# tsinghua-fib-lab/PIML

Measured on AMD Instinct MI355X. Metric: agent-pair force evals/sec + simulated steps/sec, 4096-agent GC scene, higher is better.
Workload: dtype f32

## Files before the change

### include/piml_hip_tuning.h

```cpp
#ifndef PIML_HIP_TUNING_H
#define PIML_HIP_TUNING_H

#include "piml_hip.h"

#ifdef __cplusplus
extern "C" {
#endif

int piml_timer_create(void** event);
int piml_timer_record(void* event, void* stream);
int piml_timer_elapsed_ms(void* start, void* stop, float* ms);
int piml_timer_destroy(void* event);

int piml_trace_begin(void);
int piml_trace_mark(const char* name, void* stream);
int piml_trace_end(char* names, int names_cap, float* us, int us_cap);

int piml_probe_arith(const float* rx, const float* ry, const float* hx, const float* hy,
                     float* dist, float* cosv, int n, void* stream);

long long piml_encoder_split_tiles(long long tiles);
long long piml_encoder_split_tiles_train(long long tiles);
int piml_encoder_products(int split_bf16);
int piml_rowdecoder_products(int split_bf16);
int piml_encoder_dw2(int layer_split);
int piml_encoder_fused_bwd(int on);
int piml_encoder_sums_bwd(int form);
int piml_encoder_sums_dec_slots(int on);
int piml_encoder_compact_rows(int on);
int piml_pinnsf_streams_init(void);

#ifdef __cplusplus
}
#endif
#endif
```

### piml_amd/_lib.py

```python
import ctypes
import os

import torch

_HERE = os.path.dirname(os.path.abspath(__file__))
LIB_PATH = os.environ.get('PIML_LIB') or os.path.join(_HERE, 'libpiml_hip.so')
ABI_VERSION = 35
COMPACT_MAX_AGENTS = 16384
COMPACT_SLOTS = 256

_lib = None

_i, _f, _p, _z = ctypes.c_int, ctypes.c_float, ctypes.c_void_p, ctypes.c_size_t
_ll = ctypes.c_longlong
_d = ctypes.c_double


class EncoderBranch(ctypes.Structure):
    _fields_ = [('x', _p), ('rows', _ll), ('in_dim', _i), ('k', _i),
                ('w1', _p), ('b1', _p), ('w2', _p), ('b2', _p), ('w3', _p), ('b3', _p),
                ('scale', _f), ('h1', _p), ('h2', _p), ('msgs', _p), ('g_pooled', _p), ('g_msgs', _p),
                ('g2', _p), ('g1', _p), ('g_x', _p), ('partials', _p), ('grads', _p), ('packed', _p), ('relu_mask', _p),
                ('keep_bits', _p), ('drop_state', _p), ('drop_p', _f), ('sum_a', _p), ('sum_b', _p),
                ('nbr_idx', _p), ('plan', _p)]
# ... 176 lines not shown
    'piml_train_step_tail_bwd': [_p, _ll, _p, _p, _p, _p, _ll, _p, _p, _i, _i, _i, _i, _f, _p, _p, _p, _p, _p, _f, _i, _i, _p, _p, _p, _p],
    'piml_pinnsf_epilogue_fwd': [_p, _p, _p, _z, _f, _p, _p],
    'piml_pinnsf_epilogue_bwd': [_p, _p, _z, _f, _p, _p],
    'piml_pinnsf_epilogue_ksum_fwd': [_p, _i, _p, _i, _p, _z, _f, _p, _p],
    'piml_pinnsf_epilogue_ksum_bwd': [_p, _p, _z, _f, _i, _i, _p, _p, _p, _p],
    'piml_pinnsf_epilogue_agentnorm_fwd': [_p, _p, _p, _i, _i, _f, _p, _p],
    'piml_pinnsf_epilogue_ksum_agentnorm_fwd': [_p, _i, _p, _i, _p, _i, _i, _f, _p, _p],
    'piml_pinnsf_epilogue_agentnorm_bwd': [_p, _p, _i, _i, _f, _p, _p],
    'piml_self_features_fwd': [_p, _i, _p, _p, _z, _p, _p],
    'piml_self_features_bwd': [_p, _z, _p, _p, _p, _p],
    'piml_colsum_blocks': [_z, _i],
    'piml_act_bwd_colsum': [_p, _p, _z, _i, _p, _p, _p, _p],
    'piml_sum_leading': [_p, _i, _z, _p, _p],
    'piml_act_bwd_colsum_stage1': [_p, _p, _z, _i, _p, _p, _p, _p],
    'piml_layer_reduce': [_p, _i, _z, _p, _p, _i, _i, _p, _p],
    'piml_scale_ksum_fwd': [_p, _p, _z, _i, _i, _f, _p, _p, _p, _p],
    'piml_ksum_blocks': [_z, _i],
    'piml_scale_ksum_bwd': [_p, _p, _z, _i, _i, _f, _p, _p, _p, _p],
    'piml_dropout_keep_bits': [_p, _ll, _i, _f, _i, _p, _p],
    'piml_timer_create': [ctypes.POINTER(_p)],
    'piml_timer_record': [_p, _p],
    'piml_timer_elapsed_ms': [_p, _p, ctypes.POINTER(_f)],
    'piml_timer_destroy': [_p],
    'piml_trace_begin': [],
    'piml_trace_mark': [ctypes.c_char_p, _p],
    'piml_trace_end': [ctypes.c_char_p, _i, ctypes.POINTER(_f), _i],
    'piml_probe_arith': [_p, _p, _p, _p, _p, _p, _i, _p],
    'piml_encoder_partial_floats': [],
    'piml_encoder_pack_floats': [],
    'piml_encoder_split_tiles': [_ll],
    'piml_encoder_split_tiles_train': [_ll],
    'piml_multi_copy': [ctypes.POINTER(_p), ctypes.POINTER(_p), ctypes.POINTER(_z), _i, _p],
    'piml_rollout_prologue': [_p] * 8 + [_i] * 4 + [_p] * 11 + [_p],
    'piml_rollout_losses_blocks': [_i, _i],
    'piml_rollout_losses': [_p, _p, _ll, _p, _p, _p, _p, _p, _i, _i, _i, _f, _p, _p, _p, _p, _p, _p, _p],
    'piml_rollout_losses_bwd': [_p, _p, _p, _p, _p, _p, _ll, _p, _p],
    'piml_rollout_losses_frames': [_p, _p, _ll, _p, _p, ctypes.POINTER(_p), _i, _p, _i, _i, _i, _f, _f, _f, _p, _p, _p, _p, _p, _p, _p],
    'piml_rollout_losses_frames_bwd': [_p, _p, _p, _p, _f, _f, _p, _p, _p, _ll, _p, _p],
    'piml_collision_pred_loss_blocks': [_ll, _i],
    'piml_collision_pred_loss': [ctypes.POINTER(_p), ctypes.POINTER(_p), _i, _ll, _i, _i, _p, _i, _i, _f, _p, _p, _p, _p, _p],
    'piml_collision_pred_loss_bwd': [_p, _p, _ll, _p, _p],
    'piml_adam_tickets': [],
    'piml_adam_step': [ctypes.POINTER(_p)] * 5 + [ctypes.POINTER(_ll), _i, ctypes.c_double, ctypes.c_double, ctypes.c_double, ctypes.c_double, ctypes.c_double, _p, _p],
    'piml_pointwise_losses_blocks': [_ll, _ll, _i],
    'piml_pointwise_losses': [_p, _p, _ll, _ll, _p, _ll, _f, _p, _i, _p, _p, _p, _p, _p],
    'piml_p2p_alloc': [_z, ctypes.POINTER(_p)],
    'piml_p2p_free': [_p],
    'piml_p2p_export': [_p, _p],
    'piml_p2p_open': [_p, ctypes.POINTER(_p)],
    'piml_p2p_close': [_p],
    'piml_p2p_copy': [_p, _p, _z, _p],
    'piml_allgather_state_p2p': [_p, _z, _i, _i, ctypes.POINTER(_p), ctypes.POINTER(_p), ctypes.c_uint, ctypes.c_uint, _p, _p],
    'piml_encoder_products': [_i],
    'piml_rowdecoder_products': [_i],
    'piml_encoder_dw2': [_i],
    'piml_encoder_fused_bwd': [_i],
    'piml_encoder_sums_bwd': [_i],
    'piml_encoder_sums_dec_slots': [_i],
    'piml_encoder_compact_rows': [_i],
    'piml_encoder_pack': [ctypes.POINTER(EncoderBranch), _i, _p],
    'piml_encoder_workgroups': [ctypes.POINTER(EncoderBranch), _i, ctypes.POINTER(_i)],
    'piml_encoder_fwd': [ctypes.POINTER(EncoderBranch), _i, _p],
    'piml_encoder_fwd_packed': [ctypes.POINTER(EncoderBranch), _i, _p],
    'piml_encoder_bwd': [ctypes.POINTER(EncoderBranch), _i, _p],
    'piml_encoder_bwd_acc': [ctypes.POINTER(EncoderBranch), _i, _i, _p],
    'piml_encoder_ksum': [_p, _ll, _i, _p, _p],
    'piml_decoder_pack_floats': [],
    'piml_decoder_partial_floats': [],
    'piml_decoder_workgroups': [_ll],
    'piml_decoder_fwd': [ctypes.POINTER(DecoderBranch), _i, _p, _f, _p, _p],
    'piml_decoder_bwd': [ctypes.POINTER(DecoderBranch), _i, _p, _p, _f, _p, _p],
    'piml_rowdecoder_slots': [_ll],
    'piml_rowdecoder_fwd': [ctypes.POINTER(DecoderBranch), _i, _p],
    'piml_rowdecoder_fwd_packed': [ctypes.POINTER(DecoderBranch), _i, _p],
    'piml_rowdecoder_bwd': [ctypes.POINTER(DecoderBranch), _i, _p],
    'piml_rowdecoder_bwd_acc': [ctypes.POINTER(DecoderBranch), _i, _i, _p],
    'piml_collision_head_pack_floats': [],
    'piml_collision_head_fwd': [_p, _ll, _p, _p, _p, _p, _p, _p, _p],
    'piml_head64_partial_floats': [],
    'piml_head64_slots': [_ll],
    'piml_head64_fwd': [ctypes.POINTER(Head64), _p],
    'piml_head64_bwd': [ctypes.POINTER(Head64), _p],
    'piml_head64_bwd_acc': [ctypes.POINTER(Head64), _i, _p],
    'piml_corrector_partial_floats': [_i],
    'piml_corrector_slots': [_i, _ll, _i],
    'piml_corrector_fwd': [ctypes.POINTER(Corrector), _p],
    'piml_corrector_bwd': [ctypes.POINTER(Corrector), _i, _p],
    'piml_pinnsf_pool_h2_ok': [ctypes.POINTER(EncoderBranch), _i],
    'piml_pinnsf_pool_train_ok': [ctypes.POINTER(EncoderBranch), _i],
    'piml_pinnsf_pool_msgs_ok': [ctypes.POINTER(EncoderBranch), _i],
    'piml_pinnsf_streams_init': [],
    'piml_pinnsf_pack_flush': [],
    'piml_pinnsf_slot_sums_flush': [],
    'piml_pinnsf_pack': [ctypes.POINTER(EncoderBranch), ctypes.POINTER(DecoderBranch), _i, ctypes.POINTER(CollisionHead),
                         _i, _p],
    'piml_pinnsf_fwd': [ctypes.POINTER(EncoderBranch), ctypes.POINTER(DecoderBranch), _i, ctypes.POINTER(CollisionHead),
                        _p, _f, _p, _i, _p],
    'piml_pinnsf_bwd': [ctypes.POINTER(EncoderBranch), ctypes.POINTER(DecoderBranch), _i, _p, _p, _f, _p, _i, _p],
    'piml_comm_available': [],
    'piml_comm_unique_id': [_p],
    'piml_comm_init': [ctypes.POINTER(_p), _i, _i, _p],
    'piml_comm_destroy': [_p],
    'piml_allgather_state': [_p, _p, _z, _p, _p],
    'piml_reducescatter_grad': [_p, _p, _p, _z, _p],
    'piml_allreduce_sum': [_p, _p, _z, _p],
    'piml_relfeat_fwd_self': [_p, _p, _p, _p, _i, _p, _p, _p, _i, _i, _i, _i, _i, _i, _i, _f, _f, _f, _f, _p, _p, _p, _p, _p, _p, _p],
# ... 173 lines not shown
```

### piml_amd/csrc/network.hip

```cpp
#include <cstdio>
#include <cstdlib>
#include <mutex>

#include "common.hpp"
#include "pack.hpp"
#include "reduce.hpp"
#include "stages.hpp"
#include "trace.hpp"

namespace piml {

namespace {

struct Side {
    hipStream_t s[2] = {nullptr, nullptr};
    hipEvent_t ev[6] = {};
    bool ok = false;
};

constexpr int kMaxDevices = 64;
Side g_side[kMaxDevices];
std::mutex g_mu;

int side_streams(Side** out) {
    int dev = 0;
    if (hipError_t e = hipGetDevice(&dev)) return e;
    if (dev < 0 || dev >= kMaxDevices) return hipErrorInvalidDevice;
    std::lock_guard<std::mutex> lock(g_mu);
    Side& S = g_side[dev];
    if (!S.ok) {
        for (auto& s : S.s)
            if (hipError_t e = hipStreamCreateWithFlags(&s, hipStreamNonBlocking)) return e;
        for (auto& ev : S.ev)
            if (hipError_t e = hipEventCreateWithFlags(&ev, hipEventDisableTiming)) return e;
        S.ok = true;
    }
    *out = &S;
    return hipSuccess;
}

int edge(hipStream_t from, hipStream_t to, hipEvent_t ev) {
    if (hipError_t e = hipEventRecord(ev, from)) return e;
    return hipStreamWaitEvent(to, ev, 0);
}

#define PIML_TRY(x)                                                                        \
    do {                                                                                   \
        if (int e_ = (x)) {                                                                \
            fprintf(stderr, "libpiml_hip: %s -> %d (%s:%d)\n", #x, e_, __FILE__, __LINE__); \
            return e_;                                                                     \
        }                                                                                  \
    } while (0)

}

__global__ __launch_bounds__(256) void pinnsf_pack_kernel(PackAll A) {
    __shared__ double red[256];
    pack_block(A, (int)blockIdx.x, 256, red);
}

int launch_pack(const PackAll& A, hipStream_t s) {
    hipLaunchKernelGGL(pinnsf_pack_kernel, dim3((unsigned)pack_blocks_total(A, 256)), dim3(256), 0, s, A);
    trace_mark("pinnsf_pack", s);
    return hipGetLastError();
}

__global__ __launch_bounds__(256) void pinnsf_reduce_kernel(ReduceAll A) { reduce_launch_block(A, (int)blockIdx.x); }

int launch_slot_sums(const ReduceAll& R, hipStream_t s) {
    hipLaunchKernelGGL(pinnsf_reduce_kernel, dim3((unsigned)reduce_launch_blocks(R)), dim3(256), 0, s, R);
    return hipGetLastError();
}

__global__ __launch_bounds__(256) void pinnsf_unfold_kernel(ReduceAll R) { unfold_block(R, (int)(blockIdx.y * kUnfoldBlocks + blockIdx.x)); }

static int launch_unfold_now(const ReduceAll& R, hipStream_t s) {
    if (R.nunf <= 0) return hipSuccess;
    hipLaunchKernelGGL(pinnsf_unfold_kernel, dim3(kUnfoldBlocks, (unsigned)R.nunf), dim3(256), 0, s, R);
    trace_mark("pinnsf_unfold", s);
    return hipGetLastError();
}

namespace {
struct PendingUnfold {
    ReduceAll R;
    hipStream_t stream = nullptr;
    bool valid = false, deferring = false;
};
PendingUnfold g_pending_unfold[kMaxDevices];
PendingUnfold* pending_unfold_entry() {
    int dev = 0;
    if (hipGetDevice(&dev) || dev < 0 || dev >= kMaxDevices) return nullptr;
    return &g_pending_unfold[dev];
}
bool same_unfold(const ReduceAll& a, const ReduceAll& b) {
    if (a.nunf != b.nunf) return false;
    for (int i = 0; i < a.nunf; ++i)
        if (a.unf[i].dgrads != b.unf[i].dgrads || a.unf[i].dw1_out != b.unf[i].dw1_out || a.unf[i].egrads != b.unf[i].egrads ||
            a.unf[i].w1 != b.unf[i].w1 || a.unf[i].w3 != b.unf[i].w3 || a.unf[i].b3 != b.unf[i].b3 || a.unf[i].k != b.unf[i].k ||
            a.unf[i].scale != b.unf[i].scale)
            return false;
    return true;
}
}

ReduceAll unfold_begin(const ReduceAll& R, hipStream_t s, UnfoldTail* t) {
    ReduceAll out = R;
    out.unf_blocks = 0;
    t->go = false;
    if (R.nunf <= 0) return out;
    PendingUnfold* P = pending_unfold_entry();
// ... 376 lines not shown
```

### piml_amd/csrc/reduce.hpp

```cpp
#pragma once
#include <hip/hip_runtime.h>

#include "pack.hpp"

namespace piml {

struct ReduceSet {
    const float* parts;
    float* grads;
    int slots, lanes, split, off0, off1;
    const int* dev_slots;
};
struct UnfoldSet {
    const float* dgrads;
    const float *w1, *w3, *b3;
    float scale;
    int k;
    float* dw1_out;
    float* egrads;
};
constexpr int REDUCE_SETS = 8;
struct ReduceAll {
    ReduceSet set[REDUCE_SETS];
    int nsets;
// ... 69 lines not shown
    const int y = bid / A.gx, x = bid - y * A.gx;
    const ReduceSet S = A.set[y];
    if (x * 16 < S.lanes) sum_slots_16x16_at(x, S.parts, S.grads, S.dev_slots ? *S.dev_slots : S.slots, S.lanes, S.split, S.off0, S.off1, A.accumulate != 0);
}
__device__ __forceinline__ void reduce_launch_block(const ReduceAll& A, int bid) {
    if (bid < A.unf_blocks) unfold_block(A, bid);
    else reduce_block(A, bid - A.unf_blocks);
}
__host__ __device__ inline int reduce_launch_blocks(const ReduceAll& A) { return A.unf_blocks + A.gx * A.nsets; }

struct PackAll {
    piml_encoder_branch enc[2];
    piml_decoder_branch dec[2];
    piml_collision_head head;
    int nbr, has_head;
    int has_fold;
    int skip_f32;
};
constexpr int ENC_LIVE_X3 = PACK_FLOATS - 2 * 32768;
__host__ __device__ inline int enc_set_elems(const PackAll& A) { return A.skip_f32 ? ENC_LIVE_X3 : PACK_FLOATS; }
__host__ __device__ inline int pack_elems_total(const PackAll& A) {
    return A.nbr * (enc_set_elems(A) + DEC_PACK_PLAIN) + (A.has_head ? HEAD_PACK_PLAIN : 0);
}

__device__ __forceinline__ void pack_flat(const PackAll& A, int t) {
    const int ne = enc_set_elems(A);
    for (int y = 0; y < A.nbr; ++y) {
        if (t < ne) {
            int e = t;
            if (A.skip_f32) e = t < PACK_FWD - 32768 ? t + 32768 : t + 2 * 32768;
            const piml_encoder_branch& J = A.enc[y];
            J.packed[e] = pack_value(J, e);
            return;
        }
        t -= ne;
    }
    for (int y = 0; y < A.nbr; ++y) {
        if (t < DEC_PACK_PLAIN) {
            const piml_decoder_branch& J = A.dec[y];
            J.packed[t] = dec_pack_value(J, t);
            return;
        }
        t -= DEC_PACK_PLAIN;
    }
    if (A.has_head && t < HEAD_PACK_PLAIN) A.head.packed[t] = head_pack_value(A.head, t);
}
__host__ __device__ inline int fold_sets(const PackAll& A) { return A.has_fold ? A.nbr + (A.has_head ? 1 : 0) : 0; }
__host__ __device__ inline int fold_groups_per_block(int threads) { return threads >= 512 ? threads / 512 : 1; }
__host__ __device__ inline int fold_blocks(const PackAll& A, int threads) {
    const int g = fold_groups_per_block(threads);
    return (fold_sets(A) * FOLD_GROUPS + g - 1) / g;
}
template <int CH>
__device__ __forceinline__ void fold_block(const PackAll& A, int fb, int threads, double* red) {
    const int wave = (int)threadIdx.x >> 6, lane = (int)threadIdx.x & 63;
    const int grp = fb * ((threads >> 6) / CH) + wave / CH, chunk = wave % CH;
    const int f = grp / FOLD_GROUPS, r = grp - f * FOLD_GROUPS, i = r / 3, hc = r - 3 * i;
    const bool live = f < fold_sets(A);
    const bool is_head = f >= A.nbr;
    const piml_decoder_branch& J = A.dec[is_head ? 0 : f];
    const float* w1 = is_head ? A.head.w1 : J.w1;
    const float* w3 = is_head ? A.head.fold_w3 : J.fold_w3;
    const float* b3 = is_head ? A.head.fold_b3 : J.fold_b3;
    const bool have = live && w3 != nullptr;
    double part = 0.0;
    if (have && (hc < 2 || lane == 0))
        part = fold_partial<CH>(w1 + (size_t)i * DH, hc < 2 ? w3 + 64 * hc + lane : b3, hc < 2 ? EH : 1, chunk);
    red[threadIdx.x] = part;
    __syncthreads();
    if (have && chunk == 0) {
        double sum = 0.0;
#pragma unroll
        for (int c = 0; c < CH; ++c) sum += red[threadIdx.x + 64 * c];
        if (is_head) head_fold_store(A.head, i, hc, lane, sum);
        else dec_fold_store(J, i, hc, lane, sum);
    }
}
constexpr int kPackPerThread = 4;
struct PackWork {
    PackAll A;
    int first_block;
};
__host__ __device__ inline int pack_plain_blocks(const PackAll& A, int threads) {
    return (pack_elems_total(A) + threads * kPackPerThread - 1) / (threads * kPackPerThread);
}
__device__ __forceinline__ void zrow_block(const PackAll& A, int y, int threads, double* red) {
    const piml_encoder_branch& J = A.enc[y];
    const int t = (int)threadIdx.x, parts = threads >= 512 ? 4 : 2, per = EH / parts;
    double part = 0.0;
    if (t < parts * EH) {
        const int j = t & (EH - 1), p = t >> 7;
        const float* __restrict__ wr = J.w2 + (size_t)j * EH + p * per;
        const float* __restrict__ br = J.b1 + p * per;
        for (int q0 = 0; q0 < per; q0 += 16) {
            float wv[16], bv[16];
#pragma unroll
            for (int u = 0; u < 16; ++u) { wv[u] = wr[q0 + u]; bv[u] = br[q0 + u]; }
#pragma unroll
            for (int u = 0; u < 16; ++u) part += (double)wv[u] * (double)fmaxf(bv[u], 0.f);
        }
    }
    red[t] = part;
    __syncthreads();
    if (t < EH) {
        double sum = 0.0;
        for (int p = 0; p < parts; ++p) sum += red[t + p * EH];
        J.packed[PACK_ZROW + t] = fmaxf(J.b1[t], 0.f);
        J.packed[PACK_ZROW + EH + t] = fmaxf((float)((double)J.b2[t] + sum), 0.f);
    }
}
__host__ __device__ inline int pack_blocks_total(const PackAll& A, int threads) { return pack_plain_blocks(A, threads) + fold_blocks(A, threads) + A.nbr; }
__device__ __forceinline__ void pack_block(const PackAll& A, int bid, int threads, double* red) {
    const int plain = pack_plain_blocks(A, threads);
    if (bid < plain) {
        const int total = pack_elems_total(A);
#pragma unroll
        for (int j = 0; j < kPackPerThread; ++j) {
            const int t = (bid * kPackPerThread + j) * threads + (int)threadIdx.x;
            if (t < total) pack_flat(A, t);
        }
    } else if (bid >= plain + fold_blocks(A, threads)) {
        zrow_block(A, bid - plain - fold_blocks(A, threads), threads, red);
    } else if (threads >= 512) {
        fold_block<8>(A, bid - plain, threads, red);
    } else {
        fold_block<4>(A, bid - plain, threads, red);
    }
}
int launch_pack(const PackAll& A, hipStream_t s);
int pending_pack_leave(const PackAll& A, hipStream_t s);
bool pending_pack_take(hipStream_t s, PackAll* out);
int pending_pack_flush(hipStream_t consumer);

int launch_slot_sums(const ReduceAll& R, hipStream_t s);
int pending_slot_sums_leave(const ReduceAll& R, hipStream_t s);
bool pending_slot_sums_take(hipStream_t s, ReduceAll* out);
int pending_slot_sums_flush();
bool pending_slot_sums_write(const float* grads);

}
```

### piml_amd/csrc/relfeat.hip

```cpp
#include "common.hpp"
#include "trace.hpp"
#include "reduce.hpp"
#include "../../include/piml_hip.h"

#include <cmath>
#include <cstdlib>

namespace piml {

constexpr int kTile = 4096;
constexpr int kRing = 1024;

struct RelfeatArgs {
    const float* p; const float* v; const float* a;
    const float2* hd; const float2* dest; const float2* obs;
    int ld;
    int C, N, M, f0, fcnt, kp, ko;
    float cos_p, cos_o, cut2_p, cut2_o, dthr_p, dthr_o;
    float* ped_feat; float* obs_feat; float* dest_feat; int dest_ld; int* ped_idx; int* obs_idx;
    int a_lo[2], a_hi[2];
    int flags;
    int split;
    const float* speed;
    float* zero; long zero_n;
// ... 48 lines not shown
    const int ld = A.ld;
    const int kpe = min(A.kp, A.N), koe = min(A.ko, A.M);
    const size_t row = (size_t)c * A.fcnt + fl;
    if (lane < kpe && (flags & kRfPedList)) {
        const u64 key = lists[0];
        A.ped_idx[row * kpe + lane] = key == kEmptyKey ? -1 : (int)(unsigned)key;
    }
    if (lane < kpe && (flags & kRfPedFeat)) {
        const u64 key = lists[0];
        const int j = key == kEmptyKey ? -1 : (int)(unsigned)key;
        float f0 = 0.f, f1 = 0.f, f2 = 0.f, f3 = 0.f, f4 = 0.f, f5 = 0.f;
        if (j >= 0) {
            const size_t cj = ((size_t)c * A.N + j) * ld;
            const float2 pj = *reinterpret_cast<const float2*>(A.p + cj);
            const float2 vj = *reinterpret_cast<const float2*>(A.v + cj);
            const float2 aj = *reinterpret_cast<const float2*>(A.a + cj);
            f0 = pj.x - pix; f1 = pj.y - piy;
            f2 = nan_to_zero(vj.x) - vix; f3 = nan_to_zero(vj.y) - viy;
            f4 = nan_to_zero(aj.x) - aix; f5 = nan_to_zero(aj.y) - aiy;
        }
        float2* out = reinterpret_cast<float2*>(A.ped_feat + (row * kpe + lane) * 6);
        out[0] = make_float2(f0, f1); out[1] = make_float2(f2, f3); out[2] = make_float2(f4, f5);
        A.ped_idx[row * kpe + lane] = j;
    }
    if (lane < koe && (flags & kRfObs)) {
        const u64 key = lists[1];
        const int j = key == kEmptyKey ? -1 : (int)(unsigned)key;
        float f0 = 0.f, f1 = 0.f, f2 = 0.f, f3 = 0.f, f4 = 0.f, f5 = 0.f;
        if (j >= 0) {
            const float2 oj = A.obs[j];
            f0 = oj.x - pix; f1 = oj.y - piy;
            f2 = 0.f - vix; f3 = 0.f - viy; f4 = 0.f - aix; f5 = 0.f - aiy;
        }
        float2* out = reinterpret_cast<float2*>(A.obs_feat + (row * koe + lane) * 6);
        out[0] = make_float2(f0, f1); out[1] = make_float2(f2, f3); out[2] = make_float2(f4, f5);
        A.obs_idx[row * koe + lane] = j;
    }
    if (lane == 0 && (flags & kRfDest)) {
        const float2 d = A.dest[row];
        float* df = A.dest_feat + row * A.dest_ld;
        df[0] = nan_to_zero(d.x - pix); df[1] = nan_to_zero(d.y - piy);
        if (A.speed) {
            df[2] = vi2.x; df[3] = vi2.y; df[4] = ai2.x; df[5] = ai2.y;
            df[6] = A.speed[row];
        }
    }
}

constexpr int kObsTile = 2048;

template <int WAVES, bool RES>
constexpr int relfeat_lds_bytes() { return (2 * kTile + WAVES * kRing / 2 + (RES ? 2 * kObsTile : 0)) * 4; }

template <int WAVES, bool RES>
__global__ __launch_bounds__(WAVES * 64) void relfeat_fwd_kernel(const RelfeatArgs A, const PackWork PK) {
    extern __shared__ __attribute__((aligned(16))) float rf_lds[];
    if (PK.first_block >= 0 && (int)blockIdx.x >= PK.first_block) {
        pack_block(PK.A, (int)blockIdx.x - PK.first_block, WAVES * 64, reinterpret_cast<double*>(rf_lds));
        return;
    }
    float* const agent_x = rf_lds;
    float* const agent_y = rf_lds + kTile;
    unsigned short* const ring_base = reinterpret_cast<unsigned short*>(rf_lds + 2 * kTile);
    float* const obs_x = RES ? rf_lds + 2 * kTile + WAVES * kRing / 2 : agent_x;
    float* const obs_y = RES ? obs_x + kObsTile : agent_y;

    const int lane = threadIdx.x & 63;
    const int wave = uniform((int)(threadIdx.x >> 6));
    unsigned short* ring = ring_base + wave * kRing;

    if (A.tick && blockIdx.x == 0 && threadIdx.x == 0) *A.tick += 1;
    if (A.zero)
        for (long e = (long)blockIdx.x * (WAVES * 64) + threadIdx.x; e < A.zero_n;
             e += (long)(PK.first_block >= 0 ? PK.first_block : (int)gridDim.x) * (WAVES * 64))
            A.zero[e] = 0.f;

    const int bpc = (A.fcnt + WAVES - 1) / WAVES;
    const int nb = A.C * bpc;
    const int kind = (!RES && A.split) ? ((int)blockIdx.x >= nb ? 2 : 1) : 0;
    const int bid = (int)blockIdx.x - (kind == 2 ? nb : 0);
    const int flags = kind == 1 ? (A.flags & ~kRfObs) : (kind == 2 ? kRfObs : A.flags);
    const int c = bid / bpc;
    const int fl = (bid - c * bpc) * WAVES + wave;
    const bool has = fl < A.fcnt;
    const int i = A.f0 + (has ? fl : 0);
    const size_t ci = (size_t)c * A.N + i;

    const int ld = A.ld;
    const float2 pi2 = *reinterpret_cast<const float2*>(A.p + ci * ld);
    const float pix = uniform(pi2.x), piy = uniform(pi2.y);
    const float2 vi2 = *reinterpret_cast<const float2*>(A.v + ci * ld);
    const float2 ai2 = *reinterpret_cast<const float2*>(A.a + ci * ld);
    const float vix = uniform(nan_to_zero(vi2.x)), viy = uniform(nan_to_zero(vi2.y));
    const float aix = uniform(nan_to_zero(ai2.x)), aiy = uniform(nan_to_zero(ai2.y));
    const bool alive = has && pix == pix && piy == piy;

    float hx, hy;
    if (A.hd) {
        const float2 h = A.hd[ci];
        hx = uniform(h.x); hy = uniform(h.y);
    } else {
        float hn = norm2(vix, viy);
        if (hn == 0.f) hn = hn + 0.1f;
        hx = __fdiv_rn(vix, hn); hy = __fdiv_rn(viy, hn);
    }
    const float n2c = fmaxf(norm2(hx, hy), 1e-8f);
    const float h0 = __fdiv_rn(hx, n2c), h1 = __fdiv_rn(hy, n2c);
    typedef float v2f __attribute__((ext_vector_type(2)));
    const v2f pix2 = {pix, pix}, piy2 = {piy, piy};

#ifdef PIML_RELFEAT_STATS
    int st_evals = 0, st_rounds = 0, st_ins = 0, st_cand = 0;
    unsigned long long st_t[8] = {0, 0, 0, 0, 0, 0, 0, 0};
    int st_n = 0;
    st_t[st_n++] = __builtin_amdgcn_s_memtime();
#define PIML_STAT(x) x
#else
#define PIML_STAT(x)
#endif
    const float qnan = __uint_as_float(0x7fc00000u);
    auto stage = [&](const float* __restrict__ src, int sld, int base, int tn, int tn_pad, float* tx, float* ty) {
        for (int t = threadIdx.x; t < tn_pad; t += WAVES * 64) {
            float2 q = make_float2(qnan, qnan);
            if (t < tn) q = *reinterpret_cast<const float2*>(src + (size_t)(base + t) * sld);
            tx[t] = q.x; ty[t] = q.y;
        }
    };
    if (RES) {
        const int n0 = A.a_hi[0] - A.a_lo[0];
        stage(A.p + (size_t)c * A.N * ld, ld, A.a_lo[0], n0, (n0 + 511) & ~511, agent_x, agent_y);
        stage((const float*)A.obs, 2, 0, A.M, (A.M + 511) & ~511, obs_x, obs_y);
        __syncthreads();
        PIML_STAT(if (st_n < 7) st_t[st_n++] = __builtin_amdgcn_s_memtime();)
    }
    u64 lists[2] = {kEmptyKey, kEmptyKey};
#pragma unroll 1
    for (int pass = kind == 2 ? 1 : 0; pass < (kind == 1 ? 1 : 2); ++pass) {
        const float* __restrict__ src = pass == 0 ? A.p + (size_t)c * A.N * ld : (const float*)A.obs;
        const int sld = pass == 0 ? ld : 2;
        const int cnt = pass == 0 ? A.N : A.M;
        const int k = pass == 0 ? A.kp : A.ko;
        const float cos_thr = pass == 0 ? A.cos_p : A.cos_o;
        const float dthr = pass == 0 ? A.dthr_p : A.dthr_o;
        float cut2 = pass == 0 ? A.cut2_p : A.cut2_o;

        if (pass == 1 && !(flags & kRfObs)) break;
        float* const tile_x = pass == 0 ? agent_x : obs_x;
        float* const tile_y = pass == 0 ? agent_y : obs_y;

        unsigned list_d = kEmptyDist, list_i = 0;
        unsigned kth_d = kEmptyDist, kth_i = 0;
        unsigned head = 0, tail = 0;
        if (pass == 0 && (flags & kRfInit) && alive && k > 0) {
            const int j = lane < k ? A.ped_idx[((size_t)c * A.fcnt + fl) * k + lane] : -1;
            if (j >= 0) {
                const float2 pj = *reinterpret_cast<const float2*>(src + (size_t)j * sld);
                list_d = __float_as_uint(norm2(pj.x - pix, pj.y - piy));
                list_i = (unsigned)j;
            }
            kth_d = (unsigned)__builtin_amdgcn_readlane((int)list_d, k - 1);
            kth_i = (unsigned)__builtin_amdgcn_readlane((int)list_i, k - 1);
            if (kth_d != kEmptyDist) {
                const float dk = __uint_as_float(kth_d);
                cut2 = fminf(cut2, dk * dk * 1.00000095367431640625f);
            }
        }

#pragma unroll 1
// ... 36 lines not shown
                        if (d2[u] <= cut2)
                            ring[mbcnt_add(m, tail) & (kRing - 1)] =
                                (unsigned short)(j0 + (u >> 2) * 256 + 4 * lane + (u & 3));
                        tail += (unsigned)__builtin_popcountll(m);
                    }
                }
#pragma unroll 1
                while (tail - head >= (flush ? 1u : 64u)) {
                    const unsigned n = min(64u, tail - head);
                    PIML_STAT(++st_evals; st_cand += (int)n;)
                    const bool act = (unsigned)lane < n;
                    __builtin_amdgcn_wave_barrier();
                    const int jl = act ? (int)ring[(head + lane) & (kRing - 1)] : 0;
                    head = uniform((int)(head + n));
                    const float rx = tile_x[jl] - pix, ry = tile_y[jl] - piy;
                    const float d = norm2(rx, ry);
                    const float cs = cos_sim_prenorm(rx, ry, d, h0, h1);
                    const bool ok = act && cs >= cos_thr && d <= dthr;
                    unsigned cd = ok ? __float_as_uint(d) : kEmptyDist;
#pragma unroll 1
                    for (;;) {
                        PIML_STAT(++st_rounds;)
                        const unsigned md = wave_min_u32(cd);
                        if (md > kth_d || md == kEmptyDist) break;
                        u64 tied = __builtin_amdgcn_ballot_w64(cd == md);
                        int s = __builtin_ctzll(tied);
                        int nj = __builtin_amdgcn_readlane(jl, s);
                        for (tied &= tied - 1; tied; tied &= tied - 1) {
                            const int s2 = __builtin_ctzll(tied);
                            const int j2 = __builtin_amdgcn_readlane(jl, s2);
                            if (j2 < nj) { nj = j2; s = s2; }
                        }
                        const unsigned ni = (unsigned)(base + nj);
                        if (md == kth_d && ni > kth_i) break;
                        PIML_STAT(++st_ins;)
                        list_insert(list_d, list_i, md, ni);
                        kth_d = (unsigned)__builtin_amdgcn_readlane((int)list_d, k - 1);
                        kth_i = (unsigned)__builtin_amdgcn_readlane((int)list_i, k - 1);
                        if (lane == s) cd = kEmptyDist;
                    }
                    if (kth_d != kEmptyDist) {
                        const float dk = __uint_as_float(kth_d);
                        cut2 = fminf(cut2, dk * dk * 1.00000095367431640625f);
                    }
                }
            }
        }
        }
        PIML_STAT(if (st_n < 7) st_t[st_n++] = __builtin_amdgcn_s_memtime();)
        const u64 mine = list_d == kEmptyDist ? kEmptyKey : (u64)list_i;
        if (pass == 0) lists[0] = mine; else lists[1] = mine;
    }

    if (!has) return;
#ifdef PIML_RELFEAT_STATS
    if (A.stats && lane == 0) {
        int* o = A.stats + ((size_t)c * A.fcnt + fl + (kind == 2 ? (size_t)A.C * A.fcnt : 0)) * 12;
        o[0] = st_evals; o[1] = st_rounds; o[2] = st_ins; o[3] = st_cand;
        for (int q = 0; q < 7; ++q) o[4 + q] = (int)(st_t[q] - st_t[0]);
    }
#endif

    relfeat_epilogue(A, flags, c, fl, lane, lists, pix, piy, vix, viy, aix, aiy, vi2, ai2);
}

__device__ __forceinline__ void relfeat_bwd_rows(
        int bid, const float* __restrict__ g_ped, const float* __restrict__ g_obs, const float2* __restrict__ g_destf,
        const int* __restrict__ ped_idx, const int* __restrict__ obs_idx, const float* __restrict__ p, int ld,
        const float2* __restrict__ dest, int C, int N, int f0, int fcnt, int kpe, int koe, float* g_state,
        float2* g_dest, int gld, float* __restrict__ g_speed) {
    const int lane = threadIdx.x & 63;
    const long row = (long)bid * 4 + (threadIdx.x >> 6);
    if (row >= (long)C * fcnt) return;
    const int c = (int)(row / fcnt), fl = (int)(row - (long)c * fcnt);
    const size_t ci = (size_t)c * N + f0 + fl;
    const int q = lane & 7, s0 = lane >> 3;
    float own = 0.f;
    const bool head = s0 == 0 && q < 6;
    float d_q = 0.f, p_q = 0.f, gdf = 0.f;
    if (head) {
        if (q < 2) {
            d_q = reinterpret_cast<const float*>(dest)[row * 2 + q];
            p_q = p[ci * ld + q];
            gdf = reinterpret_cast<const float*>(g_destf)[row * gld + q];
        } else if (gld == 7) {
            gdf = reinterpret_cast<const float*>(g_destf)[row * 7 + q];
        }
    }
    if (q < 6) {
        constexpr int TR = (PIML_MAX_TOPK + 7) / 8;
        int jp[TR], jo[TR];
        float gp[TR], go[TR];
#pragma unroll
        for (int t = 0; t < TR; ++t) {
            const int s = s0 + 8 * t;
            const bool inp = s < kpe, ino = s < koe;
            jp[t] = inp ? ped_idx[row * kpe + s] : -1;
            gp[t] = inp ? g_ped[(row * kpe + s) * 6 + q] : 0.f;
            jo[t] = ino ? obs_idx[row * koe + s] : -1;
            go[t] = ino ? g_obs[(row * koe + s) * 6 + q] : 0.f;
        }
#pragma unroll
        for (int t = 0; t < TR; ++t)
            if (jp[t] >= 0) {
                atomicAdd(g_state + ((size_t)c * N + jp[t]) * 6 + q, gp[t]);
                own -= gp[t];
            }
#pragma unroll
        for (int t = 0; t < TR; ++t)
            if (jo[t] >= 0) own -= go[t];
    }
    own += __shfl_xor(own, 8, 64);
    own += __shfl_xor(own, 16, 64);
    own += __shfl_xor(own, 32, 64);
    if (head) {
        if (q < 2) {
// ... 75 lines not shown
            if (ped_idx[row * kpe + s] >= 0) sum -= g_ped[(row * kpe + s) * 6 + q];
        for (int s = 0; s < koe; ++s)
            if (obs_idx[row * koe + s] >= 0) sum -= g_obs[(row * koe + s) * 6 + q];
        if (q < 2) {
            const float dq = reinterpret_cast<const float*>(dest)[row * 2 + q] - p[src * ld + q];
            const float gd = dq != dq ? 0.f : reinterpret_cast<const float*>(g_destf)[row * 2 + q];
            reinterpret_cast<float*>(g_dest)[row * 2 + q] = gd;
            sum -= gd;
        }
    }
    long long lo = 0, hi = nkeys;
    while (lo < hi) {
        const long long mid = (lo + hi) >> 1;
        if (sorted_keys[mid] < src) lo = mid + 1; else hi = mid;
    }
    for (long long e = lo; e < nkeys && sorted_keys[e] == src; ++e) sum += g_ped[order[e] * 6 + q];
    float* o = g_state + src * 6 + q;
    *o = accumulate ? *o + sum : sum;
}

__global__ void heading_kernel(const float2* __restrict__ vel, int C, int T, int N, float2* __restrict__ out) {
    const int t0 = blockIdx.x * blockDim.x + threadIdx.x;
    if (t0 >= C * N) return;
    const int c = t0 / N, i = t0 - c * N;
    const size_t base = (size_t)c * T * N + i;
    float tx = 0.f, ty = 0.f;
    for (int t = T - 1; t >= 0; --t) {
        float2 h = vel[base + (size_t)t * N];
        if (norm2(h.x, h.y) == 0.f) { h.x = tx; h.y = ty; } else { tx = h.x; ty = h.y; }
        out[base + (size_t)t * N] = h;
    }
    for (int t = 0; t < T; ++t) {
        float2 h = out[base + (size_t)t * N];
        if (norm2(h.x, h.y) == 0.f) { h.x = tx; h.y = ty; } else { tx = h.x; ty = h.y; }
        float n = norm2(h.x, h.y);
        if (n == 0.f) n = n + 0.1f;
        out[base + (size_t)t * N] = make_float2(__fdiv_rn(h.x, n), __fdiv_rn(h.y, n));
    }
}

static float dist2_cutoff(float thr) {
    if (!(thr >= 0.f)) return -1.f;
    if (std::isinf(thr)) return INFINITY;
    float x = thr * thr;
    while (sqrtf(x) > thr) x = nextafterf(x, -INFINITY);
    while (sqrtf(nextafterf(x, INFINITY)) <= thr) x = nextafterf(x, INFINITY);
    return x;
}

}

using namespace piml;

template <int W, bool R>
static void relfeat_go(dim3 grid, dim3 block, void* stream, const RelfeatArgs& A, bool forward_of_a_step = false) {
    constexpr int bytes = relfeat_lds_bytes<W, R>();
    PackWork PK;
    PK.first_block = -1;
    if (forward_of_a_step && pending_pack_take(as_stream(stream), &PK.A)) {
        PK.first_block = (int)grid.x;
        grid.x += (unsigned)pack_blocks_total(PK.A, W * 64);
    }
    relfeat_fwd_kernel<W, R><<<grid, block, bytes, as_stream(stream)>>>(A, PK);
}
template <int W>
static int relfeat_attr() {
    constexpr int bytes = relfeat_lds_bytes<W, true>();
    return (int)hipFuncSetAttribute(reinterpret_cast<const void*>(relfeat_fwd_kernel<W, true>), hipFuncAttributeMaxDynamicSharedMemorySize, bytes);
}

static int relfeat_launch(const float* position, const float* heading, const float* velocity,
                          const float* acceleration, int state_ld, const float* destination,
                          const float* obstacles, int C, int N, int M, int focal_begin,
                          int focal_count, int topk_ped, int topk_obs, float cos_thr_ped,
                          float cos_thr_obs, float dist_thr_ped, float dist_thr_obs,
                          float* ped_feat, float* obs_feat, float* dest_feat, int dest_feat_ld,
                          int32_t* ped_idx, int32_t* obs_idx, const float* speed, float* zero, long zero_n, void* stream,
                          int part = 0, long long* tick = nullptr) {
    if (C < 0 || N < 0 || M < 0 || focal_begin < 0 || focal_count < 0 || focal_begin + focal_count > N ||
        topk_ped < 0 || topk_obs < 0 || topk_ped > PIML_MAX_TOPK || topk_obs > PIML_MAX_TOPK ||
        state_ld < 2 || (state_ld & 1) || dest_feat_ld < 2)
        return hipErrorInvalidValue;
    if (C == 0 || focal_count == 0) return hipSuccess;
    const int kpe_ = topk_ped < N ? topk_ped : N, koe_ = topk_obs < M ? topk_obs : M;
    if (part < 0 || part > 2 || !position || !velocity || !acceleration || (kpe_ > 0 && !ped_idx)) return hipErrorInvalidValue;
    if (part != 2 && (!destination || !dest_feat || (M > 0 && !obstacles) || (koe_ > 0 && (!obs_feat || !obs_idx))))
        return hipErrorInvalidValue;
    if (part != 1 && kpe_ > 0 && !ped_feat) return hipErrorInvalidValue;
    RelfeatArgs A;
    A.a_lo[0] = 0; A.a_hi[0] = N; A.a_lo[1] = 0; A.a_hi[1] = 0;
    A.flags = kRfPedFeat | kRfObs | kRfDest;
    A.split = 0;
    if (part == 1) {
        A.a_lo[0] = focal_begin; A.a_hi[0] = focal_begin + focal_count;
        A.flags = kRfObs | kRfDest | kRfPedList;
    } else if (part == 2) {
        A.a_lo[0] = 0; A.a_hi[0] = focal_begin; A.a_lo[1] = focal_begin + focal_count; A.a_hi[1] = N;
        A.flags = kRfPedFeat | kRfInit;
    }
    A.p = position; A.v = velocity; A.a = acceleration; A.ld = state_ld;
    A.hd = (const float2*)heading; A.dest = (const float2*)destination; A.obs = (const float2*)obstacles;
    A.C = C; A.N = N; A.M = M; A.f0 = focal_begin; A.fcnt = focal_count;
    A.kp = topk_ped < N ? topk_ped : N; A.ko = topk_obs < M ? topk_obs : M;
    A.cos_p = cos_thr_ped; A.cos_o = cos_thr_obs;
    A.cut2_p = dist2_cutoff(dist_thr_ped); A.cut2_o = dist2_cutoff(dist_thr_obs);
    A.dthr_p = dist_thr_ped; A.dthr_o = dist_thr_obs;
    A.ped_feat = ped_feat; A.obs_feat = obs_feat; A.dest_feat = dest_feat; A.dest_ld = dest_feat_ld;
    A.ped_idx = ped_idx; A.obs_idx = obs_idx;
    A.speed = speed; A.zero = zero; A.zero_n = zero ? zero_n : 0; A.tick = tick;
    A.stats = nullptr;
#ifdef PIML_RELFEAT_STATS
    if (const char* e = getenv("PIML_RELFEAT_STATS_PTR")) A.stats = (int*)strtoull(e, nullptr, 0);
#endif
    const long rows = (long)C * focal_count;
    int waves = rows >= 16384 ? 8 : (rows >= 4096 ? 16 : (rows >= 1024 ? 8 : 4));
    if (N > kTile && rows >= 1024) waves = 8;
    if (const char* e = getenv("PIML_RELFEAT_WAVES")) waves = atoi(e);
    const int bpc = (focal_count + waves - 1) / waves;
    const dim3 grid((unsigned)(C * bpc)), block((unsigned)(waves * 64));
    static const bool res_off = getenv("PIML_RELFEAT_RESIDENT") && atoi(getenv("PIML_RELFEAT_RESIDENT")) == 0;
    const bool res = !res_off && (A.flags & kRfObs) && M > 0 && M <= kObsTile && A.a_hi[1] == A.a_lo[1] &&
                     A.a_hi[0] - A.a_lo[0] <= kTile && A.ko > 0;
    if (res) {
        static int attr = -1;
        if (attr < 0) {
            attr = relfeat_attr<16>();
            if (!attr) attr = relfeat_attr<8>();
            if (!attr) attr = relfeat_attr<4>();
        }
        if (attr) return attr;
    }
    static const bool split_off = getenv("PIML_RELFEAT_SPLIT") && atoi(getenv("PIML_RELFEAT_SPLIT")) == 0;
    if (!split_off && (A.flags & kRfObs) && M > 0 && A.ko > 0 && A.kp > 0 && (C == 1 || rows <= 4096)) {
        A.split = 1;
        const dim3 grid2(grid.x * 2);
        switch (waves) {
            case 16: relfeat_go<16, false>(grid2, block, stream, A, true); break;
            case 8: relfeat_go<8, false>(grid2, block, stream, A, true); break;
            case 4: relfeat_go<4, false>(grid2, block, stream, A, true); break;
            default: return hipErrorInvalidValue;
        }
        return hipGetLastError();
    }
    switch (waves * 2 + (res ? 1 : 0)) {
        case 33: relfeat_go<16, true>(grid, block, stream, A, true); break;
        case 32: relfeat_go<16, false>(grid, block, stream, A, true); break;
        case 17: relfeat_go<8, true>(grid, block, stream, A, true); break;
        case 16: relfeat_go<8, false>(grid, block, stream, A, true); break;
        case 9: relfeat_go<4, true>(grid, block, stream, A, true); break;
        case 8: relfeat_go<4, false>(grid, block, stream, A, true); break;
        default: return hipErrorInvalidValue;
    }
    return hipGetLastError();
}

PIML_API int piml_relfeat_fwd(const float* position, const float* heading, const float* velocity,
                              const float* acceleration, int state_ld, const float* destination,
                              const float* obstacles, int C, int N, int M, int focal_begin,
                              int focal_count, int topk_ped, int topk_obs, float cos_thr_ped,
                              float cos_thr_obs, float dist_thr_ped, float dist_thr_obs,
                              float* ped_feat, float* obs_feat, float* dest_feat, int dest_feat_ld,
                              int32_t* ped_idx, int32_t* obs_idx, void* stream) {
    return relfeat_launch(position, heading, velocity, acceleration, state_ld, destination, obstacles, C, N, M, focal_begin,
                          focal_count, topk_ped, topk_obs, cos_thr_ped, cos_thr_obs, dist_thr_ped, dist_thr_obs, ped_feat,
                          obs_feat, dest_feat, dest_feat_ld, ped_idx, obs_idx, nullptr, nullptr, 0, stream);
}

PIML_API int piml_relfeat_fwd_self(const float* position, const float* heading, const float* velocity,
                                   const float* acceleration, int state_ld, const float* destination, const float* obstacles,
                                   const float* desired_speed, int C, int N, int M, int focal_begin, int focal_count,
                                   int topk_ped, int topk_obs, float cos_thr_ped, float cos_thr_obs, float dist_thr_ped,
                                   float dist_thr_obs, float* ped_feat, float* obs_feat, float* self_features, int32_t* ped_idx,
                                   int32_t* obs_idx, float* g_state_zero, void* stream) {
    if (C > 0 && focal_count > 0 && (!desired_speed || !self_features)) return hipErrorInvalidValue;
    return relfeat_launch(position, heading, velocity, acceleration, state_ld, destination, obstacles, C, N, M, focal_begin,
                          focal_count, topk_ped, topk_obs, cos_thr_ped, cos_thr_obs, dist_thr_ped, dist_thr_obs, ped_feat,
                          obs_feat, self_features, 7, ped_idx, obs_idx, desired_speed, g_state_zero, (long)C * N * 6, stream);
}

PIML_API int piml_relfeat_bwd_self(const float* g_ped_feat, const float* g_obs_feat, const float* g_self, const int32_t* ped_idx,
                                   const int32_t* obs_idx, const float* position, int state_ld, const float* destination, int C,
                                   int N, int focal_begin, int focal_count, int kp_eff, int ko_eff, float* g_state,
                                   float* g_destination, float* g_speed, void* stream) {
    if (C < 0 || N < 0 || focal_begin < 0 || focal_count < 0 || focal_begin + focal_count > N || kp_eff < 0 || ko_eff < 0 ||
        state_ld < 2 || (state_ld & 1))
        return hipErrorInvalidValue;
    if (C == 0 || focal_count == 0) return hipSuccess;
    if (!g_self || !position || !destination || !g_state || !g_destination || (kp_eff > 0 && (!g_ped_feat || !ped_idx)) ||
        (ko_eff > 0 && (!g_obs_feat || !obs_idx)))
        return hipErrorInvalidValue;
    return relfeat_bwd_self_launch(g_ped_feat, g_obs_feat, g_self, ped_idx, obs_idx, position, state_ld, destination, C, N, focal_begin,
                                   focal_count, kp_eff, ko_eff, g_state, g_destination, g_speed, stream);
}

PIML_API int piml_relfeat_fwd_tick(const float* position, const float* heading, const float* velocity,
                                   const float* acceleration, int state_ld, const float* destination,
                                   const float* obstacles, int C, int N, int M, int focal_begin,
                                   int focal_count, int topk_ped, int topk_obs, float cos_thr_ped,
                                   float cos_thr_obs, float dist_thr_ped, float dist_thr_obs,
                                   float* ped_feat, float* obs_feat, float* dest_feat, int dest_feat_ld,
                                   int32_t* ped_idx, int32_t* obs_idx, long long* tick, void* stream) {
    return relfeat_launch(position, heading, velocity, acceleration, state_ld, destination, obstacles, C, N, M, focal_begin,
                          focal_count, topk_ped, topk_obs, cos_thr_ped, cos_thr_obs, dist_thr_ped, dist_thr_obs, ped_feat,
// ... 113 lines not shown
```

Baseline: 244.2 billion.

## Let obstacle relfeat workgroups absorb pack blocks as a tail, cap waves with pack

Adds an optional pack form in which the weight-pack blocks are no longer appended as extra workgroups. Instead, obstacle-kind workgroups of the split relfeat kernel run them in a strided loop after their own epilogue. By default it now also drops 16-wave launches to 8 waves whenever a pack is pending, and adds a waves-per-EU occupancy hint to the kernel. The aim is to hide pack work in idle tails and improve occupancy, at the cost of extra syncs and longer obstacle workgroups. The tail form is off unless an environment variable or the setter enables it.

```diff
diff --git a/include/piml_hip_tuning.h b/include/piml_hip_tuning.h
--- a/include/piml_hip_tuning.h
+++ b/include/piml_hip_tuning.h
@@ -28,6 +28,10 @@
 int piml_encoder_sums_bwd(int form);
 int piml_encoder_sums_dec_slots(int on);
 int piml_encoder_compact_rows(int on);
+int piml_relfeat_pack_form(int form);
+int piml_relfeat_pack_plan(int form, int waves, int obstacle_workgroups, int nbr, int has_head, int has_fold, int skip_f32,
+                           int* pack_blocks, int* share);
+int piml_relfeat_pack_tail_blocks(int b, int nb, int total, int* out, int cap);
 int piml_pinnsf_streams_init(void);
 
 #ifdef __cplusplus
diff --git a/piml_amd/_lib.py b/piml_amd/_lib.py
--- a/piml_amd/_lib.py
+++ b/piml_amd/_lib.py
@@ -252,6 +252,9 @@
     'piml_p2p_copy': [_p, _p, _z, _p],
     'piml_allgather_state_p2p': [_p, _z, _i, _i, ctypes.POINTER(_p), ctypes.POINTER(_p), ctypes.c_uint, ctypes.c_uint, _p, _p],
     'piml_encoder_products': [_i],
+    'piml_relfeat_pack_form': [_i],
+    'piml_relfeat_pack_plan': [_i, _i, _i, _i, _i, _i, _i, ctypes.POINTER(_i), ctypes.POINTER(_i)],
+    'piml_relfeat_pack_tail_blocks': [_i, _i, _i, ctypes.POINTER(_i), _i],
     'piml_rowdecoder_products': [_i],
     'piml_encoder_dw2': [_i],
     'piml_encoder_fused_bwd': [_i],
diff --git a/piml_amd/csrc/network.hip b/piml_amd/csrc/network.hip
--- a/piml_amd/csrc/network.hip
+++ b/piml_amd/csrc/network.hip
@@ -56,7 +56,7 @@
 
 __global__ __launch_bounds__(256) void pinnsf_pack_kernel(PackAll A) {
     __shared__ double red[256];
-    pack_block(A, (int)blockIdx.x, 256, red);
+    pack_block(A, (int)blockIdx.x, 256, red, (int)threadIdx.x);
 }
 
 int launch_pack(const PackAll& A, hipStream_t s) {
diff --git a/piml_amd/csrc/reduce.hpp b/piml_amd/csrc/reduce.hpp
--- a/piml_amd/csrc/reduce.hpp
+++ b/piml_amd/csrc/reduce.hpp
@@ -145,8 +145,8 @@
     return (fold_sets(A) * FOLD_GROUPS + g - 1) / g;
 }
 template <int CH>
-__device__ __forceinline__ void fold_block(const PackAll& A, int fb, int threads, double* red) {
-    const int wave = (int)threadIdx.x >> 6, lane = (int)threadIdx.x & 63;
+__device__ __forceinline__ void fold_block(const PackAll& A, int fb, int threads, double* red, int tid) {
+    const int wave = tid >> 6, lane = tid & 63;
     const int grp = fb * ((threads >> 6) / CH) + wave / CH, chunk = wave % CH;
     const int f = grp / FOLD_GROUPS, r = grp - f * FOLD_GROUPS, i = r / 3, hc = r - 3 * i;
     const bool live = f < fold_sets(A);
@@ -159,12 +159,12 @@
     double part = 0.0;
     if (have && (hc < 2 || lane == 0))
         part = fold_partial<CH>(w1 + (size_t)i * DH, hc < 2 ? w3 + 64 * hc + lane : b3, hc < 2 ? EH : 1, chunk);
-    red[threadIdx.x] = part;
+    red[tid] = part;
     __syncthreads();
     if (have && chunk == 0) {
         double sum = 0.0;
 #pragma unroll
-        for (int c = 0; c < CH; ++c) sum += red[threadIdx.x + 64 * c];
+        for (int c = 0; c < CH; ++c) sum += red[tid + 64 * c];
         if (is_head) head_fold_store(A.head, i, hc, lane, sum);
         else dec_fold_store(J, i, hc, lane, sum);
     }
@@ -173,13 +173,17 @@
 struct PackWork {
     PackAll A;
     int first_block;
-};
+    int tail_stride;
+};
+__host__ __device__ inline int pack_tail_first(int b) { return b; }
+__host__ __device__ inline int pack_tail_stride(int nb) { return nb; }
+__host__ __device__ inline int pack_tail_share(int nb, int total) { return nb > 0 ? (total + nb - 1) / nb : total; }
 __host__ __device__ inline int pack_plain_blocks(const PackAll& A, int threads) {
     return (pack_elems_total(A) + threads * kPackPerThread - 1) / (threads * kPackPerThread);
 }
-__device__ __forceinline__ void zrow_block(const PackAll& A, int y, int threads, double* red) {
+__device__ __forceinline__ void zrow_block(const PackAll& A, int y, int threads, double* red, int tid) {
     const piml_encoder_branch& J = A.enc[y];
-    const int t = (int)threadIdx.x, parts = threads >= 512 ? 4 : 2, per = EH / parts;
+    const int t = tid, parts = threads >= 512 ? 4 : 2, per = EH / parts;
     double part = 0.0;
     if (t < parts * EH) {
         const int j = t & (EH - 1), p = t >> 7;
@@ -203,21 +207,21 @@
     }
 }
 __host__ __device__ inline int pack_blocks_total(const PackAll& A, int threads) { return pack_plain_blocks(A, threads) + fold_blocks(A, threads) + A.nbr; }
-__device__ __forceinline__ void pack_block(const PackAll& A, int bid, int threads, double* red) {
+__device__ __forceinline__ void pack_block(const PackAll& A, int bid, int threads, double* red, int tid) {
     const int plain = pack_plain_blocks(A, threads);
     if (bid < plain) {
         const int total = pack_elems_total(A);
 #pragma unroll
         for (int j = 0; j < kPackPerThread; ++j) {
-            const int t = (bid * kPackPerThread + j) * threads + (int)threadIdx.x;
+            const int t = (bid * kPackPerThread + j) * threads + tid;
             if (t < total) pack_flat(A, t);
         }
     } else if (bid >= plain + fold_blocks(A, threads)) {
-        zrow_block(A, bid - plain - fold_blocks(A, threads), threads, red);
+        zrow_block(A, bid - plain - fold_blocks(A, threads), threads, red, tid);
     } else if (threads >= 512) {
-        fold_block<8>(A, bid - plain, threads, red);
+        fold_block<8>(A, bid - plain, threads, red, tid);
     } else {
-        fold_block<4>(A, bid - plain, threads, red);
+        fold_block<4>(A, bid - plain, threads, red, tid);
     }
 }
 int launch_pack(const PackAll& A, hipStream_t s);
diff --git a/piml_amd/csrc/relfeat.hip b/piml_amd/csrc/relfeat.hip
--- a/piml_amd/csrc/relfeat.hip
+++ b/piml_amd/csrc/relfeat.hip
@@ -124,11 +124,32 @@
 template <int WAVES, bool RES>
 constexpr int relfeat_lds_bytes() { return (2 * kTile + WAVES * kRing / 2 + (RES ? 2 * kObsTile : 0)) * 4; }
 
+#ifdef PIML_RELFEAT_STATS
+__device__ __forceinline__ int stat_xcc() {
+    int id;
+    asm volatile("s_getreg_b32 %0, hwreg(HW_REG_XCC_ID)" : "=s"(id));
+    return id & 15;
+}
+__device__ __forceinline__ void stat_pack_block(const RelfeatArgs& A, int pb, unsigned long long t0, unsigned long long rt0) {
+    if (A.stats && threadIdx.x == 0) {
+        int* o = A.stats + (size_t)2 * A.C * A.fcnt * 12 + (size_t)pb * 4;
+        o[0] = (int)(unsigned)rt0; o[1] = (int)(unsigned)__builtin_amdgcn_s_memrealtime();
+        o[2] = (int)(__builtin_amdgcn_s_memtime() - t0); o[3] = (int)blockIdx.x;
+    }
+}
+#endif
+
 template <int WAVES, bool RES>
-__global__ __launch_bounds__(WAVES * 64) void relfeat_fwd_kernel(const RelfeatArgs A, const PackWork PK) {
+__global__ __launch_bounds__(WAVES * 64) __attribute__((amdgpu_waves_per_eu(RES ? 1 : (WAVES == 4 ? 4 : 7)))) void relfeat_fwd_kernel(const RelfeatArgs A, const PackWork PK) {
     extern __shared__ __attribute__((aligned(16))) float rf_lds[];
     if (PK.first_block >= 0 && (int)blockIdx.x >= PK.first_block) {
-        pack_block(PK.A, (int)blockIdx.x - PK.first_block, WAVES * 64, reinterpret_cast<double*>(rf_lds));
+#ifdef PIML_RELFEAT_STATS
+        const unsigned long long pk_t0 = __builtin_amdgcn_s_memtime(), pk_rt0 = __builtin_amdgcn_s_memrealtime();
+#endif
+        pack_block(PK.A, (int)blockIdx.x - PK.first_block, WAVES * 64, reinterpret_cast<double*>(rf_lds), (int)threadIdx.x);
+#ifdef PIML_RELFEAT_STATS
+        stat_pack_block(A, (int)blockIdx.x - PK.first_block, pk_t0, pk_rt0);
+#endif
         return;
     }
     float* const agent_x = rf_lds;
@@ -186,6 +207,7 @@
     unsigned long long st_t[8] = {0, 0, 0, 0, 0, 0, 0, 0};
     int st_n = 0;
     st_t[st_n++] = __builtin_amdgcn_s_memtime();
+    const unsigned long long st_rt0 = __builtin_amdgcn_s_memrealtime();
 #define PIML_STAT(x) x
 #else
 #define PIML_STAT(x)
@@ -328,16 +350,35 @@
         if (pass == 0) lists[0] = mine; else lists[1] = mine;
     }
 
-    if (!has) return;
+    if (has) {
 #ifdef PIML_RELFEAT_STATS
-    if (A.stats && lane == 0) {
-        int* o = A.stats + ((size_t)c * A.fcnt + fl + (kind == 2 ? (size_t)A.C * A.fcnt : 0)) * 12;
-        o[0] = st_evals; o[1] = st_rounds; o[2] = st_ins; o[3] = st_cand;
-        for (int q = 0; q < 7; ++q) o[4 + q] = (int)(st_t[q] - st_t[0]);
-    }
+        if (A.stats && lane == 0) {
+            int* o = A.stats + ((size_t)c * A.fcnt + fl + (kind == 2 ? (size_t)A.C * A.fcnt : 0)) * 12;
+            o[0] = st_evals; o[1] = st_rounds; o[2] = st_ins; o[3] = st_cand;
+            for (int q = 0; q < 5; ++q) o[4 + q] = (int)(st_t[q] - st_t[0]);
+            o[9] = (int)(unsigned)st_rt0; o[10] = (int)(unsigned)__builtin_amdgcn_s_memrealtime();
+            o[11] = stat_xcc();
+        }
 #endif
-
-    relfeat_epilogue(A, flags, c, fl, lane, lists, pix, piy, vix, viy, aix, aiy, vi2, ai2);
+        relfeat_epilogue(A, flags, c, fl, lane, lists, pix, piy, vix, viy, aix, aiy, vi2, ai2);
+    }
+
+    if (!RES && kind == 2 && PK.tail_stride > 0) {
+        const int total = pack_blocks_total(PK.A, WAVES * 64);
+#pragma unroll 1
+        for (int pb = pack_tail_first(bid); pb < total; pb += pack_tail_stride(PK.tail_stride)) {
+            __syncthreads();
+#ifdef PIML_RELFEAT_STATS
+            const unsigned long long pk_t0 = __builtin_amdgcn_s_memtime(), pk_rt0 = __builtin_amdgcn_s_memrealtime();
+#endif
+            int tid = (int)threadIdx.x;
+            asm volatile("" : "+v"(tid));
+            pack_block(PK.A, pb, WAVES * 64, reinterpret_cast<double*>(rf_lds), tid);
+#ifdef PIML_RELFEAT_STATS
+            stat_pack_block(A, pb, pk_t0, pk_rt0);
+#endif
+        }
+    }
 }
 
 __device__ __forceinline__ void relfeat_bwd_rows(
@@ -519,16 +560,52 @@
 
 using namespace piml;
 
+static int g_pack_form = getenv("PIML_RELFEAT_PACK_FORM") ? atoi(getenv("PIML_RELFEAT_PACK_FORM")) == 1 : 0;
+
+static bool pack_takes_tail(int form, bool split, int obstacle_workgroups) { return form == 1 && split && obstacle_workgroups > 0; }
+
 template <int W, bool R>
-static void relfeat_go(dim3 grid, dim3 block, void* stream, const RelfeatArgs& A, bool forward_of_a_step = false) {
+static void relfeat_go(dim3 grid, dim3 block, void* stream, const RelfeatArgs& A, const PackAll* pack) {
     constexpr int bytes = relfeat_lds_bytes<W, R>();
     PackWork PK;
     PK.first_block = -1;
-    if (forward_of_a_step && pending_pack_take(as_stream(stream), &PK.A)) {
-        PK.first_block = (int)grid.x;
-        grid.x += (unsigned)pack_blocks_total(PK.A, W * 64);
+    PK.tail_stride = 0;
+    if (pack) {
+        PK.A = *pack;
+        const int blocks = pack_blocks_total(PK.A, W * 64), nb = (int)grid.x / 2;
+        if (pack_takes_tail(g_pack_form, !R && A.split, nb)) {
+            PK.tail_stride = nb;
+        } else {
+            PK.first_block = (int)grid.x;
+            grid.x += (unsigned)blocks;
+        }
     }
     relfeat_fwd_kernel<W, R><<<grid, block, bytes, as_stream(stream)>>>(A, PK);
+}
+
+PIML_API int piml_relfeat_pack_form(int form) {
+    const int old = g_pack_form;
+    if (form == 0 || form == 1) g_pack_form = form;
+    return old;
+}
+
+PIML_API int piml_relfeat_pack_plan(int form, int waves, int obstacle_workgroups, int nbr, int has_head, int has_fold, int skip_f32,
+                                    int* pack_blocks, int* share) {
+    if ((waves != 4 && waves != 8 && waves != 16) || nbr < 0 || nbr > 2 || form < 0 || form > 1) return -1;
+    PackAll P{};
+    P.nbr = nbr; P.has_head = has_head != 0; P.has_fold = has_fold != 0; P.skip_f32 = skip_f32 != 0;
+    const int blocks = pack_blocks_total(P, waves * 64);
+    if (pack_blocks) *pack_blocks = blocks;
+    if (share) *share = pack_tail_share(obstacle_workgroups, blocks);
+    return pack_takes_tail(form, true, obstacle_workgroups) ? 1 : 0;
+}
+
+PIML_API int piml_relfeat_pack_tail_blocks(int b, int nb, int total, int* out, int cap) {
+    if (b < 0 || nb <= 0 || b >= nb || total < 0) return -1;
+    int n = 0;
+    for (int pb = pack_tail_first(b); pb < total; pb += pack_tail_stride(nb), ++n)
+        if (out && n < cap) out[n] = pb;
+    return n;
 }
 template <int W>
 static int relfeat_attr() {
@@ -582,7 +659,15 @@
     const long rows = (long)C * focal_count;
     int waves = rows >= 16384 ? 8 : (rows >= 4096 ? 16 : (rows >= 1024 ? 8 : 4));
     if (N > kTile && rows >= 1024) waves = 8;
+    PackAll pack_desc;
+    const bool has_pack = pending_pack_take(as_stream(stream), &pack_desc);
+    const PackAll* pack = has_pack ? &pack_desc : nullptr;
+    if (has_pack && waves == 16) waves = 8;
     if (const char* e = getenv("PIML_RELFEAT_WAVES")) waves = atoi(e);
+    if (waves != 4 && waves != 8 && waves != 16) {
+        if (has_pack) pending_pack_leave(pack_desc, as_stream(stream));
+        return hipErrorInvalidValue;
+    }
     const int bpc = (focal_count + waves - 1) / waves;
     const dim3 grid((unsigned)(C * bpc)), block((unsigned)(waves * 64));
     static const bool res_off = getenv("PIML_RELFEAT_RESIDENT") && atoi(getenv("PIML_RELFEAT_RESIDENT")) == 0;
@@ -595,27 +680,30 @@
             if (!attr) attr = relfeat_attr<8>();
             if (!attr) attr = relfeat_attr<4>();
         }
-        if (attr) return attr;
+        if (attr) {
+            if (has_pack) pending_pack_leave(pack_desc, as_stream(stream));
+            return attr;
+        }
     }
     static const bool split_off = getenv("PIML_RELFEAT_SPLIT") && atoi(getenv("PIML_RELFEAT_SPLIT")) == 0;
     if (!split_off && (A.flags & kRfObs) && M > 0 && A.ko > 0 && A.kp > 0 && (C == 1 || rows <= 4096)) {
         A.split = 1;
         const dim3 grid2(grid.x * 2);
         switch (waves) {
-            case 16: relfeat_go<16, false>(grid2, block, stream, A, true); break;
-            case 8: relfeat_go<8, false>(grid2, block, stream, A, true); break;
-            case 4: relfeat_go<4, false>(grid2, block, stream, A, true); break;
+            case 16: relfeat_go<16, false>(grid2, block, stream, A, pack); break;
+            case 8: relfeat_go<8, false>(grid2, block, stream, A, pack); break;
+            case 4: relfeat_go<4, false>(grid2, block, stream, A, pack); break;
             default: return hipErrorInvalidValue;
         }
         return hipGetLastError();
     }
     switch (waves * 2 + (res ? 1 : 0)) {
-        case 33: relfeat_go<16, true>(grid, block, stream, A, true); break;
-        case 32: relfeat_go<16, false>(grid, block, stream, A, true); break;
-        case 17: relfeat_go<8, true>(grid, block, stream, A, true); break;
-        case 16: relfeat_go<8, false>(grid, block, stream, A, true); break;
-        case 9: relfeat_go<4, true>(grid, block, stream, A, true); break;
-        case 8: relfeat_go<4, false>(grid, block, stream, A, true); break;
+        case 33: relfeat_go<16, true>(grid, block, stream, A, pack); break;
+        case 32: relfeat_go<16, false>(grid, block, stream, A, pack); break;
+        case 17: relfeat_go<8, true>(grid, block, stream, A, pack); break;
+        case 16: relfeat_go<8, false>(grid, block, stream, A, pack); break;
+        case 9: relfeat_go<4, true>(grid, block, stream, A, pack); break;
+        case 8: relfeat_go<4, false>(grid, block, stream, A, pack); break;
         default: return hipErrorInvalidValue;
     }
     return hipGetLastError();
```

Result: faster. 249.4 billion (median of 6 runs) (+2.1%).
